# reginald-mclean/mtrl

Measured on AMD Instinct MI355X. Metric: SAC gradient-steps/sec, MT50 width-2048 batch=128/task, 1/2/4/8 MI355X, higher is better.
Workload: dtype fp32 (2xfp16 split, per-tensor power-of-two scaled, 3 fp16 MFMA products, fp32-accurate); 1 GPU; MT50 MTMHSAC-v2 width=2048 (experiments/width_scaling/mt50_mtmhsac_v2_2048.py); num_tasks=50, width=2048, batch_per_task=128, global_batch=6400, parallelism=single, precision=split2h, exec=eager

## Files before the change

### mtrl_amd/csrc/gemm_common.h

```cpp
#pragma once
#include "kernels.h"

namespace mtsac {

struct GemmSlice {
  const float* A;
  const float* B;
  float* C;
  float* db;
  int K, ldc, z;
};

template <bool TA, bool TB>
__device__ inline GemmSlice gemm_slice(const GemmParams& p) {
  GemmSlice s;
  const int S = p.splits > 1 ? p.splits : 1;
  const int zz = blockIdx.z, z = zz / S, sp = zz - z * S;
  const int k0 = sp * p.kchunk;
  s.z = z;
  s.K = S > 1 ? min(p.kchunk, p.K - k0) : p.K;
  s.A = p.A + z * p.sA + (TA ? (long long)k0 * p.lda : (long long)k0);
  s.B = p.B + z * p.sB + (TB ? (long long)k0 : (long long)k0 * p.ldb);
  if (S > 1) {
    const long long slab = (long long)p.M * p.N;
    s.C = p.ws + zz * slab;
    s.ldc = p.N;
    s.db = p.db ? p.ws + (long long)gridDim.z * slab + (long long)zz * p.N : nullptr;
  } else {
    s.C = p.C + z * p.sC;
    s.ldc = p.ldc;
    s.db = p.db ? p.db + z * p.sDb : nullptr;
  }
  return s;
}

typedef float f32x16_t __attribute__((ext_vector_type(16)));
typedef __bf16 bf16x4_t __attribute__((ext_vector_type(4)));

struct TileOut {
  float* C;
  long long ldc;
  const float* bias;
  const float* mask;
  long long ldm;
  __bf16* Cp;
  long long ldcp, pC;
  int M, N;
  bool vec;
  bool h2;
  float unscale, oscale;
};

typedef _Float16 f16x8 __attribute__((ext_vector_type(8)));

__host__ __device__ inline long long frag_off(long long n, long long k, long long ldk) {
  return (((n >> 4) * (ldk >> 5) + (k >> 5)) << 9) + (((n & 15) + 16 * ((k >> 3) & 3)) << 3) + (k & 7);
}
typedef _Float16 f16x4 __attribute__((ext_vector_type(4)));

__device__ inline void split2h_dev(float x, float s, _Float16& h, _Float16& l) {
  const float y = x * s;
  h = (_Float16)y;
  l = (_Float16)(y - (float)h);
  if (x > 0.f && h == (_Float16)0.f && l == (_Float16)0.f) l = __builtin_bit_cast(_Float16, (unsigned short)1);
}

__device__ inline int plane_exp(float bound) {
  bound *= 1.00390625f;
  if (!(bound > 0.f) || !(bound < 3.0e38f)) return 0;
  int ex;
  (void)frexpf(bound, &ex);
  return min(100, max(-100, 15 - ex));
}

__device__ inline float block_max_val(float m, float* scratch) {
#pragma unroll
  for (int o = 32; o > 0; o >>= 1) m = fmaxf(m, __shfl_xor(m, o));
  __syncthreads();
  if ((threadIdx.x & 63) == 0) scratch[threadIdx.x >> 6] = m;
  __syncthreads();
  float r = 0.f;
  for (int w = 0; w < (int)(blockDim.x + 63) / 64; ++w) r = fmaxf(r, scratch[w]);
  __syncthreads();
  return r;
}

__device__ inline float block_max_of(const float* __restrict__ v, int n, float* scratch) {
  float m = 0.f;
  for (int i = threadIdx.x; i < n; i += blockDim.x) m = fmaxf(m, v[i]);
#pragma unroll
  for (int o = 32; o > 0; o >>= 1) m = fmaxf(m, __shfl_xor(m, o));
  __syncthreads();
  if ((threadIdx.x & 63) == 0) scratch[threadIdx.x >> 6] = m;
  __syncthreads();
  float r = 0.f;
  for (int w = 0; w < (int)(blockDim.x + 63) / 64; ++w) r = fmaxf(r, scratch[w]);
  __syncthreads();
  return r;
}

__device__ inline float exp2i(int e) { return __builtin_bit_cast(float, (unsigned)(127 + e) << 23); }

__device__ inline float rec_max(const PlaneRec* r, int n, float* scratch) {
  if (r == nullptr) return 0.f;
  if (n <= 0) return exp2i(15 - r->e);
  return block_max_of(r->amax, n, scratch);
}

__device__ inline int gemm_out_exp(const SplitGemmParams& p, float* scratch) {
  const float ma = rec_max(p.ra, p.na, scratch);
  const float mb = rec_max(p.rb, p.nb, scratch);
  return plane_exp(p.kmul * ma * mb + (p.bias_in_b ? mb : 0.f));
}

__device__ inline void split3_dev(float x, __bf16& h, __bf16& m, __bf16& l) {
  h = (__bf16)x;
  const float r1 = x - (float)h;
  m = (__bf16)r1;
  l = (__bf16)(r1 - (float)m);
}

template <int EPI>
__device__ inline void store_tile32(const f32x16_t& acc, float* scr, int lane, int row0, int col0, const TileOut& o,
                                    float& omx) {
  const int lr = lane & 31, lh = lane >> 5;
#pragma unroll
  for (int r = 0; r < 16; ++r) scr[((r & 3) + 8 * (r >> 2) + 4 * lh) * 36 + lr] = acc[r];
  __builtin_amdgcn_fence(__ATOMIC_RELEASE, "wavefront");
  __builtin_amdgcn_wave_barrier();
  __builtin_amdgcn_fence(__ATOMIC_ACQUIRE, "wavefront");
  const int c4 = 4 * (lane & 7);
  const int col = col0 + c4;
#pragma unroll
  for (int q = 0; q < 4; ++q) {
    const int rr = (lane >> 3) + 8 * q;
    const int row = row0 + rr;
    if (row >= o.M) continue;
    float4 v = *reinterpret_cast<const float4*>(scr + rr * 36 + c4);
    float e[4] = {v.x, v.y, v.z, v.w};
    if (o.h2) {
#pragma unroll
      for (int j = 0; j < 4; ++j) e[j] *= o.unscale;
    }
    if (o.vec && col + 3 < o.N) {
      if (EPI == EPI_BIAS_RELU) {
        const float4 b = *reinterpret_cast<const float4*>(o.bias + col);
        e[0] = fmaxf(e[0] + b.x, 0.f); e[1] = fmaxf(e[1] + b.y, 0.f);
        e[2] = fmaxf(e[2] + b.z, 0.f); e[3] = fmaxf(e[3] + b.w, 0.f);
      }
      if (EPI == EPI_RELU_MASK) {
        const float4 mk = *reinterpret_cast<const float4*>(o.mask + (long long)row * o.ldm + col);
        e[0] = mk.x > 0.f ? e[0] : 0.f; e[1] = mk.y > 0.f ? e[1] : 0.f;
        e[2] = mk.z > 0.f ? e[2] : 0.f; e[3] = mk.w > 0.f ? e[3] : 0.f;
      }
      if (o.C) *reinterpret_cast<float4*>(o.C + (long long)row * o.ldc + col) = make_float4(e[0], e[1], e[2], e[3]);
      if (o.Cp && o.h2) {
        f16x4 h, l;
#pragma unroll
        for (int j = 0; j < 4; ++j) {
          _Float16 a, b;
          split2h_dev(e[j], o.oscale, a, b);
          h[j] = a; l[j] = b;
          omx = fmaxf(omx, fabsf(e[j]));
        }
        __bf16* cp = o.Cp + (long long)row * o.ldcp + col;
        *reinterpret_cast<f16x4*>(cp) = h;
        *reinterpret_cast<f16x4*>(cp + o.pC) = l;
      } else if (o.Cp) {
        bf16x4_t h, m, l;
#pragma unroll
        for (int j = 0; j < 4; ++j) {
          __bf16 a, b, c;
          split3_dev(e[j], a, b, c);
          h[j] = a; m[j] = b; l[j] = c;
        }
        __bf16* cp = o.Cp + (long long)row * o.ldcp + col;
        *reinterpret_cast<bf16x4_t*>(cp) = h;
        *reinterpret_cast<bf16x4_t*>(cp + o.pC) = m;
        *reinterpret_cast<bf16x4_t*>(cp + 2 * o.pC) = l;
      }
    } else {
#pragma unroll
      for (int j = 0; j < 4; ++j) {
        const int cc = col + j;
        if (cc >= o.N) continue;
        float x = e[j];
        if (EPI == EPI_BIAS_RELU) x = fmaxf(x + o.bias[cc], 0.f);
        if (EPI == EPI_RELU_MASK) x = o.mask[(long long)row * o.ldm + cc] > 0.f ? x : 0.f;
        if (o.C) o.C[(long long)row * o.ldc + cc] = x;
        if (o.Cp && o.h2) {
          _Float16 a, b;
          split2h_dev(x, o.oscale, a, b);
          omx = fmaxf(omx, fabsf(x));
          reinterpret_cast<_Float16*>(o.Cp)[(long long)row * o.ldcp + cc] = a;
          reinterpret_cast<_Float16*>(o.Cp)[(long long)row * o.ldcp + cc + o.pC] = b;
        } else if (o.Cp) {
          __bf16 a, b, c;
          split3_dev(x, a, b, c);
          __bf16* cp = o.Cp + (long long)row * o.ldcp + cc;
          cp[0] = a;
          cp[o.pC] = b;
          cp[2 * o.pC] = c;
        }
      }
    }
  }
  __builtin_amdgcn_fence(__ATOMIC_RELEASE, "wavefront");
  __builtin_amdgcn_wave_barrier();
  __builtin_amdgcn_fence(__ATOMIC_ACQUIRE, "wavefront");
}

}
```

### mtrl_amd/csrc/gemm_x3p_impl.h

```cpp
#pragma once
#include <algorithm>

#include "gemm_common.h"

namespace mtsac {

typedef f32x16_t f32x16;
typedef __bf16 bf16x8 __attribute__((ext_vector_type(8)));
typedef short i16x4 __attribute__((ext_vector_type(4)));
typedef short i16x8 __attribute__((ext_vector_type(8)));

namespace x3pk {

constexpr int BK = 32;

typedef __attribute__((address_space(3))) void lds_void;

__device__ inline void glds16(const void* src, unsigned lds_addr) {
  asm volatile("s_mov_b32 m0, %1\n\ts_nop 0\n\tglobal_load_lds_dwordx4 %0, off" ::"v"(src),
               "s"(__builtin_amdgcn_readfirstlane(lds_addr))
               : "memory");
}
template <int R, bool KM, int KS, int NP = 3>
struct Oper {
  static constexpr int PLANE = R * KS * 2;
  static constexpr int BYTES = NP * PLANE;
  static constexpr int NJ = NP * PLANE / 1024;
  static constexpr int ROWB = KM ? 2 * R : 2 * KS;
  static constexpr int RPI = 1024 / ROWB;
  static constexpr int LPR = ROWB / 16;
  static constexpr int PER_PLANE = NJ / NP;
  static_assert(!KM || LPR >= 16, "k-major swizzle needs >= 16 chunks per row");

  __device__ static inline int pchunk(int irow, int c) {
    if (KM) return c ^ (4 * (irow & 3));
    return KS == 32 ? (c ^ ((irow >> 2) & 3)) : (c ^ ((irow >> 3) & 1));
  }

  __device__ static inline void dma(const __bf16* __restrict__ base, long long ld, long long ps, int r0, int nrows,
                                    int k0, unsigned lds, int first, int stride) {
#pragma unroll
    for (int j = first; j < NJ; j += stride) dma_one(base, ld, ps, r0, nrows, k0, lds, j);
  }

  __device__ static inline void dma_one(const __bf16* __restrict__ base, long long ld, long long ps, int r0, int nrows,
                                        int k0, unsigned lds, int j) {
    const int lane = threadIdx.x & 63;
    {
      const int q = j / PER_PLANE;
      const int ib = (j % PER_PLANE) * RPI;
      const int irow = ib + lane / LPR;
      const int c = pchunk(irow, lane % LPR);
      const __bf16* src;
      if (KM) {
        int col = r0 + 8 * c;
        const int last = ((nrows + 7) & ~7) - 8;
        col = col < last ? col : last;
        src = base + q * ps + (long long)(k0 + irow) * ld + col;
      } else {
        int row = r0 + irow;
        row = row < nrows ? row : nrows - 1;
        src = base + q * ps + (long long)row * ld + k0 + 8 * c;
      }
      glds16(src, lds + q * PLANE + ib * ROWB);
    }
  }

  __device__ static inline const __bf16* dma_src(const __bf16* __restrict__ base, long long ld, long long ps, int r0,
                                                 int nrows, int k0, int j) {
    static_assert(KM, "k-major images only");
    const int lane = threadIdx.x & 63;
    const int q = j / PER_PLANE;
    const int irow = (j % PER_PLANE) * RPI + lane / LPR;
    int col = r0 + 8 * pchunk(irow, lane % LPR);
    const int last = ((nrows + 7) & ~7) - 8;
    col = col < last ? col : last;
    return base + q * ps + (long long)(k0 + irow) * ld + col;
  }
  __device__ static inline unsigned dma_dst(int j) { return (j / PER_PLANE) * PLANE + (j % PER_PLANE) * RPI * ROWB; }

  __device__ static inline bf16x8 frag(const char* lds, int q, int rb, int ks, int lane) {
    const char* pl = lds + q * PLANE;
    if (!KM) {
      const int r = rb + (lane & 31);
      const int o = r * ROWB + 16 * pchunk(r, (KS / 8 == 4 ? 2 * ks : 0) + (lane >> 5));
      return *reinterpret_cast<const bf16x8*>(pl + o);
    } else {
      const int G = lane >> 4, i = lane & 15, qq = i >> 2, p = i & 3;
      const int m = rb + 16 * (G & 1) + 4 * p;
      const int c = m >> 3, inb = 8 * (p & 1);
      const int k0 = 16 * ks + 8 * (G >> 1) + qq;
      const int o0 = k0 * ROWB + 16 * pchunk(k0, c) + inb;
      const int o1 = (k0 + 4) * ROWB + 16 * pchunk(k0 + 4, c) + inb;
      const i16x4 lo = __builtin_amdgcn_ds_read_tr16_b64_v4i16((__attribute__((address_space(3))) i16x4*)(pl + o0));
      const i16x4 hi = __builtin_amdgcn_ds_read_tr16_b64_v4i16((__attribute__((address_space(3))) i16x4*)(pl + o1));
      const i16x8 v = {lo[0], lo[1], lo[2], lo[3], hi[0], hi[1], hi[2], hi[3]};
      return __builtin_bit_cast(bf16x8, v);
    }
  }
};

template <int BM_, int BN_, int WM_, int WN_, int STAGES_, int KS_, int TAG = 0>
struct Geo {
  static constexpr int BM = BM_, BN = BN_, WM = WM_, WN = WN_, STAGES = STAGES_, KS = KS_;
  static constexpr int NW = WM * WN, NTH = 64 * NW;
  static constexpr int TI = BM / WM / 32, TJ = BN / WN / 32;
};

template <int V>
struct IntC {
  static constexpr int value = V;
};

template <class G, bool AKM, bool BKM, int EPI, bool PLANES_OUT, int NP = 3, bool FIN = false, bool PIPE = false,
          int ABL = 0>
__global__ __launch_bounds__(G::NTH, 1) void gemm_x3p_kernel(SplitGemmParams p) {
  using OA = Oper<G::BM, AKM, G::KS, NP>;
  using OB = Oper<G::BN, BKM, G::KS, NP>;
  constexpr int STAGE = OA::BYTES + OB::BYTES;
  constexpr int DMA_LO = (OA::NJ + OB::NJ) / G::NW, DMA_X = (OA::NJ + OB::NJ) % G::NW;
  constexpr int RING = PIPE ? (NP == 2 ? 6 : 4) : G::STAGES;
  static_assert(RING * STAGE + (FIN ? 16 : 0) <= 160 * 1024, "LDS");
  __shared__ __attribute__((aligned(16))) char smem[RING * STAGE + (FIN ? 16 : 0)];
  char* lds = smem;
  const unsigned lds_base = (unsigned)(unsigned long long)(lds_void*)smem;

  const int ny = (p.N + G::BN - 1) / G::BN, nx = (p.M + G::BM - 1) / G::BM;
  const int t = threadIdx.x, lane = t & 63;
  const int wave = __builtin_amdgcn_readfirstlane(t >> 6);
  const int wm = (wave % G::WM) * (G::BM / G::WM), wn = (wave / G::WM) * (G::BN / G::WN);
  const int fb = (G::NW - (OA::NJ % G::NW) + wave) % G::NW;
  constexpr int PIECES = DMA_LO + (DMA_X ? 1 : 0);
  constexpr int SLOTS = (G::KS / 16) * G::TI * G::TJ;

  f32x16 acc[G::TI][G::TJ];

  auto kloop = [&](const __bf16* __restrict__ A, const __bf16* __restrict__ B, int m0, int n0, int nk) {
    auto stage = [&](int s, int k0) {
      const unsigned st = lds_base + s * STAGE;
      OA::dma(A, p.lda, p.pA, m0, p.M, k0, st, wave, G::NW);
      OB::dma(B, p.ldb, p.pB, n0, p.N, k0, st + OA::BYTES, fb, G::NW);
    };
    auto piece = [&](int s, int k0, int q) {
      const unsigned st = lds_base + s * STAGE;
      const int jg = wave + q * G::NW;
      if (jg < OA::NJ)
        OA::dma_one(A, p.lda, p.pA, m0, p.M, k0, st, jg);
      else if (jg - OA::NJ < OB::NJ)
        OB::dma_one(B, p.ldb, p.pB, n0, p.N, k0, st + OA::BYTES, jg - OA::NJ);
    };
#pragma unroll
    for (int i = 0; i < G::TI; ++i)
#pragma unroll
      for (int j = 0; j < G::TJ; ++j) acc[i][j] = f32x16{0};

#pragma unroll
    for (int s = 0; s < G::STAGES - 1; ++s)
      if (s < nk) stage(s, s * G::KS);

    for (int kt = 0; kt < nk; ++kt) {
      const int younger = min(G::STAGES - 2, nk - 1 - kt);
      const bool more = DMA_X != 0 && wave < DMA_X;
      if (younger >= 3) {
        if (more) asm volatile("s_waitcnt vmcnt(%0)" ::"n"(3 * (DMA_LO + 1)) : "memory");
        else asm volatile("s_waitcnt vmcnt(%0)" ::"n"(3 * DMA_LO) : "memory");
      } else if (younger == 2) {
        if (more) asm volatile("s_waitcnt vmcnt(%0)" ::"n"(2 * (DMA_LO + 1)) : "memory");
        else asm volatile("s_waitcnt vmcnt(%0)" ::"n"(2 * DMA_LO) : "memory");
      } else if (younger == 1) {
        if (more) asm volatile("s_waitcnt vmcnt(%0)" ::"n"(DMA_LO + 1) : "memory");
        else asm volatile("s_waitcnt vmcnt(%0)" ::"n"(DMA_LO) : "memory");
      } else {
        asm volatile("s_waitcnt vmcnt(0)" ::: "memory");
      }
      __builtin_amdgcn_s_barrier();
      __builtin_amdgcn_sched_barrier(0);
      const bool refill = kt + G::STAGES - 1 < nk && !(p.dbg & 1);
      const int rs = (kt + G::STAGES - 1) % G::STAGES, rk = (kt + G::STAGES - 1) * G::KS;
      if (refill && (p.dbg & 8)) stage(rs, rk);
      const bool spread = refill && !(p.dbg & 8);
      const char* cur = lds + (kt % G::STAGES) * STAGE;
#pragma unroll
      for (int ks = 0; ks < G::KS / 16; ++ks) {
        bf16x8 a[G::TI][NP], b[G::TJ][NP];
#pragma unroll
        for (int i = 0; i < G::TI; ++i)
#pragma unroll
          for (int q = 0; q < NP; ++q) a[i][q] = OA::frag(cur, q, wm + 32 * i, ks, lane);
#pragma unroll
        for (int j = 0; j < G::TJ; ++j)
#pragma unroll
          for (int q = 0; q < NP; ++q) b[j][q] = OB::frag(cur + OA::BYTES, q, wn + 32 * j, ks, lane);
        if (p.dbg & 2) {
#pragma unroll
          for (int i = 0; i < G::TI; ++i)
#pragma unroll
            for (int j = 0; j < G::TJ; ++j) acc[i][j][0] += (float)a[i][0][0] + (float)b[j][2][7];
          if (spread && ks == 0)
#pragma unroll
            for (int q = 0; q < PIECES; ++q) piece(rs, rk, q);
          continue;
        }
#pragma unroll
        for (int i = 0; i < G::TI; ++i)
#pragma unroll
          for (int j = 0; j < G::TJ; ++j) {
            const int slot = (ks * G::TI + i) * G::TJ + j;
            if (spread) {
#pragma unroll
              for (int q = slot * PIECES / SLOTS; q < (slot + 1) * PIECES / SLOTS; ++q) piece(rs, rk, q);
            }
            f32x16 c = acc[i][j];
            if constexpr (NP == 2) {
              typedef _Float16 h8 __attribute__((ext_vector_type(8)));
              c = __builtin_amdgcn_mfma_f32_32x32x16_f16(__builtin_bit_cast(h8, a[i][0]), __builtin_bit_cast(h8, b[j][1]), c, 0, 0, 0);
              c = __builtin_amdgcn_mfma_f32_32x32x16_f16(__builtin_bit_cast(h8, a[i][1]), __builtin_bit_cast(h8, b[j][0]), c, 0, 0, 0);
              c = __builtin_amdgcn_mfma_f32_32x32x16_f16(__builtin_bit_cast(h8, a[i][0]), __builtin_bit_cast(h8, b[j][0]), c, 0, 0, 0);
              acc[i][j] = c;
              continue;
            }
            if constexpr (NP == 3) {
              c = __builtin_amdgcn_mfma_f32_32x32x16_bf16(a[i][1], b[j][1], c, 0, 0, 0);
              c = __builtin_amdgcn_mfma_f32_32x32x16_bf16(a[i][0], b[j][2], c, 0, 0, 0);
              c = __builtin_amdgcn_mfma_f32_32x32x16_bf16(a[i][2], b[j][0], c, 0, 0, 0);
              c = __builtin_amdgcn_mfma_f32_32x32x16_bf16(a[i][0], b[j][1], c, 0, 0, 0);
              c = __builtin_amdgcn_mfma_f32_32x32x16_bf16(a[i][1], b[j][0], c, 0, 0, 0);
            }
            c = __builtin_amdgcn_mfma_f32_32x32x16_bf16(a[i][0], b[j][0], c, 0, 0, 0);
            acc[i][j] = c;
          }
      }
    }
  };

  auto epilogue = [&](int z, int zz, bool raw, int m0, int n0) {
    TileOut o{};
    if (raw) {
      o.C = p.ws + (long long)zz * p.M * p.N;
      o.ldc = p.N;
    } else {
      o.C = p.C ? p.C + z * p.sC : nullptr;
      o.ldc = p.ldc;
    }
    o.bias = (EPI == EPI_BIAS_RELU) ? p.bias + z * p.sBias : nullptr;
    o.mask = (EPI == EPI_RELU_MASK) ? p.mask + z * p.sMask : nullptr;
    o.ldm = p.ldm;
    o.Cp = (PLANES_OUT && !raw) ? p.Cp + z * p.sCp : nullptr;
    o.ldcp = p.ldcp;
    o.pC = p.pC;
    o.M = p.M;
    o.N = p.N;
    o.vec = (p.N % 4 == 0) && (o.ldc % 4 == 0) && (EPI != EPI_RELU_MASK || p.ldm % 4 == 0) &&
            (!PLANES_OUT || p.ldcp % 4 == 0);
    o.h2 = NP == 2;
    o.unscale = o.oscale = 1.f;
    __builtin_amdgcn_s_barrier();
    float* mscr = reinterpret_cast<float*>(smem) + G::NW * (32 * 36);
    if constexpr (NP == 2) {
      o.unscale = exp2i(-p.ra->e) * exp2i(-p.rb->e);
      if (o.Cp) {
        const int ec = gemm_out_exp(p, mscr);
        o.oscale = exp2i(ec);
        if (blockIdx.x == 0 && t == 0) p.rc->e = ec;
      }
    }
    float omx = 0.f;
    float* scr = reinterpret_cast<float*>(smem) + wave * (32 * 36);
#pragma unroll
    for (int i = 0; i < G::TI; ++i)
#pragma unroll
      for (int j = 0; j < G::TJ; ++j) store_tile32<EPI>(acc[i][j], scr, lane, m0 + wm + 32 * i, n0 + wn + 32 * j, o, omx);
    if constexpr (NP == 2) {
      if (o.Cp) {
        const float m = block_max_val(omx, mscr);
        if (t == 0 && blockIdx.x < PLANE_REC_PARTS) p.rc->amax[blockIdx.x] = m;
      }
    }
  };

  int lin = blockIdx.x;
  if (!(p.dbg & 4)) {
    const int n = gridDim.x, q8 = n / 8, r8 = n % 8, x = lin % 8;
    lin = (x < r8 ? x * (q8 + 1) : r8 * (q8 + 1) + (x - r8) * q8) + lin / 8;
  }
  const int S = p.splits > 1 ? p.splits : 1;
  const int sp0 = FIN ? lin % S : 0;
  if (FIN) lin /= S;
  const int by = lin % ny, bx = (lin / ny) % nx;
  const int z = FIN ? lin / (ny * nx) : lin / (ny * nx) / S;
  const int sp = FIN ? sp0 : lin / (ny * nx) - z * S;
  const int zz = z * S + sp;
  const long long k0 = (long long)sp * p.kchunk;
  const int nks = (S > 1 ? min(p.kchunk, p.K - (int)k0) : p.K) / G::KS;
  const int m0 = bx * G::BM, n0 = by * G::BN;
  if constexpr (PIPE) {
    static_assert(AKM && BKM && G::KS == 16 && (NP == 2 || NP == 3), "the k-major weight-grad form");
    static_assert(OA::NJ % G::NW == 0, "every wave's first pieces are A's, the rest B's");
    static_assert(RING >= 3, "ring depth");
    constexpr int D = RING;
    constexpr int QA = OA::NJ / G::NW;
    struct Frag {
      bf16x8 a[G::TI][NP], b[G::TJ][NP];
    };
    const __bf16* __restrict__ A = p.A + z * p.sA + k0 * p.lda;
    const __bf16* __restrict__ B = p.B + z * p.sB + k0 * p.ldb;
    const int nk = nks;
    const bool extra = DMA_X != 0 && wave < DMA_X;
    const __bf16* src[PIECES];
    unsigned dst[PIECES];
#pragma unroll
    for (int q = 0; q < PIECES; ++q) {
      const int jg = wave + q * G::NW;
      if (q < QA) {
        src[q] = OA::dma_src(A, p.lda, p.pA, m0, p.M, D * G::KS, jg);
        dst[q] = OA::dma_dst(jg);
      } else {
        const int jb = jg - OA::NJ < OB::NJ ? jg - OA::NJ : 0;
        src[q] = OB::dma_src(B, p.ldb, p.pB, n0, p.N, D * G::KS, jb);
        dst[q] = OA::BYTES + OB::dma_dst(jb);
      }
    }
    const long long inc_a = (long long)G::KS * p.lda, inc_b = (long long)G::KS * p.ldb;
    auto piece = [&](unsigned st, int q) __attribute__((always_inline)) {
      if (q < DMA_LO || extra) glds16(src[q], st + dst[q]);
      src[q] += q < QA ? inc_a : inc_b;
    };
    auto wait_c = [&](auto Y) __attribute__((always_inline)) {
      constexpr int y = decltype(Y)::value;
      if (DMA_X != 0 && extra) asm volatile("s_waitcnt vmcnt(%0)" ::"n"(y * (DMA_LO + 1)) : "memory");
      else asm volatile("s_waitcnt vmcnt(%0)" ::"n"(y * DMA_LO) : "memory");
    };
    auto wait_rt = [&](int y) __attribute__((always_inline)) {
      if constexpr (D - 1 >= 5) if (y >= 5) return wait_c(IntC<5>{});
      if constexpr (D - 1 >= 4) if (y == 4) return wait_c(IntC<4>{});
      if constexpr (D - 1 >= 3) if (y == 3) return wait_c(IntC<3>{});
      if (y == 2) return wait_c(IntC<2>{});
      if (y == 1) return wait_c(IntC<1>{});
      return wait_c(IntC<0>{});
    };
    static_assert(D - 1 <= 5 && (D - 1) * (DMA_LO + 1) < 64, "vmcnt range");
    auto load = [&](Frag& f, const char* st) __attribute__((always_inline)) {
#pragma unroll
      for (int i = 0; i < G::TI; ++i)
#pragma unroll
        for (int q = 0; q < NP; ++q) f.a[i][q] = OA::frag(st, q, wm + 32 * i, 0, lane);
#pragma unroll
      for (int j = 0; j < G::TJ; ++j)
#pragma unroll
        for (int q = 0; q < NP; ++q) f.b[j][q] = OB::frag(st + OA::BYTES, q, wn + 32 * j, 0, lane);
    };

#pragma unroll
    for (int i = 0; i < G::TI; ++i)
#pragma unroll
      for (int j = 0; j < G::TJ; ++j) acc[i][j] = f32x16{0};

#pragma unroll
    for (int s = 0; s < D; ++s)
      if (s < nk) {
        const unsigned st = lds_base + s * STAGE;
        OA::dma(A, p.lda, p.pA, m0, p.M, s * G::KS, st, wave, G::NW);
        OB::dma(B, p.ldb, p.pB, n0, p.N, s * G::KS, st + OA::BYTES, fb, G::NW);
      }
    wait_rt(min(D, nk) - 1);
    __builtin_amdgcn_s_barrier();
    __builtin_amdgcn_sched_barrier(0);
    Frag f0, f1;
    load(f0, lds);

    int slot = 0, nslot = 1 % D;
    auto step = [&](int kt, Frag& cur, Frag& nxt, auto MAINC) __attribute__((always_inline)) {
      constexpr bool MAIN = decltype(MAINC)::value != 0;
      if constexpr (MAIN) wait_c(IntC<D - 2>{});
      else wait_rt(min(D - 2, max(0, nk - 2 - kt)));
      asm volatile("s_waitcnt lgkmcnt(0)" ::: "memory");
      __builtin_amdgcn_s_barrier();
      __builtin_amdgcn_sched_barrier(0);
      const bool refill = !(ABL & 1) && (MAIN || kt + D < nk);
      const bool pre = MAIN || kt + 1 < nk;
      const unsigned rst = lds_base + slot * STAGE;
      const char* nst = lds + nslot * STAGE;
      if ((ABL & 8) && refill) {
#pragma unroll
        for (int q = 0; q < PIECES; ++q) piece(rst, q);
      }
#pragma unroll
      for (int i = 0; i < G::TI; ++i)
#pragma unroll
        for (int j = 0; j < G::TJ; ++j) {
          const int g = i * G::TJ + j;
          if (!(ABL & 8) && refill) {
#pragma unroll
            for (int q = g * PIECES / SLOTS; q < (g + 1) * PIECES / SLOTS; ++q) piece(rst, q);
          }
          if constexpr ((ABL & 2) != 0) {
            acc[i][j][0] += (float)cur.a[i][0][0] + (float)cur.b[j][NP - 1][7];
          } else {
            f32x16 c = acc[i][j];
            if constexpr (NP == 2) {
              typedef _Float16 h8 __attribute__((ext_vector_type(8)));
              c = __builtin_amdgcn_mfma_f32_32x32x16_f16(__builtin_bit_cast(h8, cur.a[i][0]), __builtin_bit_cast(h8, cur.b[j][1]), c, 0, 0, 0);
              c = __builtin_amdgcn_mfma_f32_32x32x16_f16(__builtin_bit_cast(h8, cur.a[i][1]), __builtin_bit_cast(h8, cur.b[j][0]), c, 0, 0, 0);
              c = __builtin_amdgcn_mfma_f32_32x32x16_f16(__builtin_bit_cast(h8, cur.a[i][0]), __builtin_bit_cast(h8, cur.b[j][0]), c, 0, 0, 0);
            } else {
              c = __builtin_amdgcn_mfma_f32_32x32x16_bf16(cur.a[i][1], cur.b[j][1], c, 0, 0, 0);
              c = __builtin_amdgcn_mfma_f32_32x32x16_bf16(cur.a[i][0], cur.b[j][2], c, 0, 0, 0);
              c = __builtin_amdgcn_mfma_f32_32x32x16_bf16(cur.a[i][2], cur.b[j][0], c, 0, 0, 0);
              c = __builtin_amdgcn_mfma_f32_32x32x16_bf16(cur.a[i][0], cur.b[j][1], c, 0, 0, 0);
              c = __builtin_amdgcn_mfma_f32_32x32x16_bf16(cur.a[i][1], cur.b[j][0], c, 0, 0, 0);
              c = __builtin_amdgcn_mfma_f32_32x32x16_bf16(cur.a[i][0], cur.b[j][0], c, 0, 0, 0);
            }
            acc[i][j] = c;
          }
          if (g == 0 && pre) load(nxt, nst);
          __builtin_amdgcn_sched_barrier(0);
        }
      slot = nslot;
      nslot = nslot + 1 == D ? 0 : nslot + 1;
    };
    int kt = 0;
    for (; kt + D + 1 < nk; kt += 2) {
      step(kt, f0, f1, IntC<1>{});
      step(kt + 1, f1, f0, IntC<1>{});
    }
    for (; kt < nk; kt += 2) {
      step(kt, f0, f1, IntC<0>{});
      if (kt + 1 < nk) step(kt + 1, f1, f0, IntC<0>{});
    }
  } else {
    kloop(p.A + z * p.sA + (AKM ? k0 * p.lda : k0), p.B + z * p.sB + (BKM ? k0 * p.ldb : k0), m0, n0, nks);
  }
  epilogue(z, zz, S > 1, m0, n0);
  if constexpr (FIN) {
    asm volatile("s_waitcnt vmcnt(0)" ::: "memory");
    __syncthreads();
    int* last = reinterpret_cast<int*>(smem + RING * STAGE);
    const int tile = lin;
    if (t == 0) {
      __builtin_amdgcn_fence(__ATOMIC_RELEASE, "agent");
      asm volatile("s_waitcnt vmcnt(0)" ::: "memory");
      const int tk = __hip_atomic_fetch_add(p.cnt + tile, 1, __ATOMIC_RELAXED, __HIP_MEMORY_SCOPE_AGENT);
      const int me = tk == S - 1;
      if (me) __hip_atomic_store(p.cnt + tile, 0, __ATOMIC_RELAXED, __HIP_MEMORY_SCOPE_AGENT);
      *last = me;
    }
    __syncthreads();
    if (*last == 0) return;
    if (t == 0) {
      __builtin_amdgcn_fence(__ATOMIC_ACQUIRE, "agent");
      asm volatile("s_waitcnt vmcnt(0)" ::: "memory");
    }
    __syncthreads();
    const long long slab = (long long)p.M * p.N;
    const float* w = p.ws + (long long)z * S * slab;
    float* c = p.C + z * p.sC;
    constexpr int Q = G::BN / 4;
    constexpr int U = 8;
    static_assert(G::BM * Q % (G::NTH * U) == 0, "reduce tiling");
    for (int e0 = t; e0 < G::BM * Q; e0 += G::NTH * U) {
      float4 a[U];
      long long off[U];
      bool ok[U];
#pragma unroll
      for (int u = 0; u < U; ++u) {
        const int e = e0 + u * G::NTH, r = m0 + e / Q, cc = n0 + 4 * (e % Q);
        ok[u] = r < p.M && cc < p.N;
        off[u] = (long long)r * p.N + cc;
        if (ok[u]) a[u] = *reinterpret_cast<const float4*>(w + off[u]);
      }
      for (int s = 1; s < S; ++s) {
#pragma unroll
        for (int u = 0; u < U; ++u)
          if (ok[u]) {
            const float4 v = *reinterpret_cast<const float4*>(w + s * slab + off[u]);
            a[u].x += v.x; a[u].y += v.y; a[u].z += v.z; a[u].w += v.w;
          }
      }
#pragma unroll
      for (int u = 0; u < U; ++u)
        if (ok[u]) {
          const int e = e0 + u * G::NTH, r = m0 + e / Q, cc = n0 + 4 * (e % Q);
          *reinterpret_cast<float4*>(c + (long long)r * p.ldc + cc) = a[u];
        }
    }
  }
}

using GeoSmall = Geo<128, 128, 2, 2, 3, 32>;
using GeoWide = Geo<256, 128, 4, 2, 2, 32>;
using GeoWide16 = Geo<256, 128, 4, 2, 4, 16>;
using GeoBig16 = Geo<256, 256, 2, 4, 3, 16>;
using GeoSmall16 = Geo<128, 128, 2, 2, 3, 16>;
using GeoBig16In = Geo<256, 256, 2, 4, 3, 16, 1>;
using GeoTall224 = Geo<224, 256, 1, 8, 3, 16>;
using GeoTall224In = Geo<224, 256, 1, 8, 3, 16, 1>;

template <class G, bool AKM, bool BKM, int NP>
void launch_x3p_np(const SplitGemmParams& p, int epi, dim3 grid, hipStream_t st) {
  const bool planes = p.Cp != nullptr;
  const dim3 block(G::NTH);
  if constexpr (AKM && BKM && NP == 3 && G::STAGES * (G::BM + G::BN) * G::KS * 2 * 3 + 16 <= 160 * 1024) {
    if (epi == EPI_STORE && !planes && p.cnt != nullptr && p.splits > 1) {
      hipLaunchKernelGGL((gemm_x3p_kernel<G, true, true, EPI_STORE, false, 3, true>), grid, block, 0, st, p);
      return;
    }
  }
  if constexpr (AKM && BKM && (NP == 2 || NP == 3) && G::BM == 256 && G::BN == 128 && G::WM == 4 && G::WN == 2 &&
                G::KS == 16) {
    if (epi == EPI_STORE && !planes && !(p.dbg & 16)) {
      const int abl = NP != 2 ? 0 : (p.dbg & 1) ? 1 : (p.dbg & 2) ? 2 : (p.dbg & 8);
      if (abl == 1) hipLaunchKernelGGL((gemm_x3p_kernel<G, true, true, EPI_STORE, false, NP, false, true, NP == 2 ? 1 : 0>), grid, block, 0, st, p);
      else if (abl == 2) hipLaunchKernelGGL((gemm_x3p_kernel<G, true, true, EPI_STORE, false, NP, false, true, NP == 2 ? 2 : 0>), grid, block, 0, st, p);
      else if (abl == 8) hipLaunchKernelGGL((gemm_x3p_kernel<G, true, true, EPI_STORE, false, NP, false, true, NP == 2 ? 8 : 0>), grid, block, 0, st, p);
      else hipLaunchKernelGGL((gemm_x3p_kernel<G, true, true, EPI_STORE, false, NP, false, true, 0>), grid, block, 0, st, p);
      return;
    }
  }
  if (epi == EPI_BIAS_RELU) {
    if (planes) hipLaunchKernelGGL((gemm_x3p_kernel<G, AKM, BKM, EPI_BIAS_RELU, true, NP>), grid, block, 0, st, p);
    else hipLaunchKernelGGL((gemm_x3p_kernel<G, AKM, BKM, EPI_BIAS_RELU, false, NP>), grid, block, 0, st, p);
  } else if (epi == EPI_RELU_MASK) {
    if (planes) hipLaunchKernelGGL((gemm_x3p_kernel<G, AKM, BKM, EPI_RELU_MASK, true, NP>), grid, block, 0, st, p);
    else hipLaunchKernelGGL((gemm_x3p_kernel<G, AKM, BKM, EPI_RELU_MASK, false, NP>), grid, block, 0, st, p);
  } else {
    if (planes) hipLaunchKernelGGL((gemm_x3p_kernel<G, AKM, BKM, EPI_STORE, true, NP>), grid, block, 0, st, p);
    else hipLaunchKernelGGL((gemm_x3p_kernel<G, AKM, BKM, EPI_STORE, false, NP>), grid, block, 0, st, p);
  }
}

template <class G, bool AKM, bool BKM>
void launch_x3p_v(const SplitGemmParams& p, int epi, dim3 grid, hipStream_t st) {
  if (p.np == 1) launch_x3p_np<G, AKM, BKM, 1>(p, epi, grid, st);
  else if (p.np == 2) launch_x3p_np<G, AKM, BKM, 2>(p, epi, grid, st);
  else launch_x3p_np<G, AKM, BKM, 3>(p, epi, grid, st);
}

template <class G, int MASK>
void launch_forms(const SplitGemmParams& p, int epi, dim3 grid, hipStream_t st) {
  const int form = (p.a_kmajor ? 1 : 0) | (p.b_kmajor ? 2 : 0);
#define X3P_FORM(F, AK, BK)                      \
  if constexpr (((MASK >> F) & 1) != 0)          \
    if (form == F) {                             \
      launch_x3p_v<G, AK, BK>(p, epi, grid, st); \
      return;                                    \
    }
  X3P_FORM(0, false, false)
  X3P_FORM(1, true, false)
  X3P_FORM(2, false, true)
  X3P_FORM(3, true, true)
#undef X3P_FORM
}

}

#define X3P_UNIT(NAME, GEO, MASK)                                           \
  void NAME(const SplitGemmParams& p, int epi, dim3 grid, hipStream_t st) { \
    x3pk::launch_forms<x3pk::GEO, MASK>(p, epi, grid, st);                  \
  }
void x3p_unit_g0(const SplitGemmParams&, int, dim3, hipStream_t);
void x3p_unit_g1(const SplitGemmParams&, int, dim3, hipStream_t);
void x3p_unit_g2(const SplitGemmParams&, int, dim3, hipStream_t);
void x3p_unit_g3f0(const SplitGemmParams&, int, dim3, hipStream_t);
void x3p_unit_g3f1(const SplitGemmParams&, int, dim3, hipStream_t);
void x3p_unit_g3f2(const SplitGemmParams&, int, dim3, hipStream_t);
void x3p_unit_g3f3(const SplitGemmParams&, int, dim3, hipStream_t);
void x3p_unit_g4(const SplitGemmParams&, int, dim3, hipStream_t);
void x3p_unit_g3in(const SplitGemmParams&, int, dim3, hipStream_t);
void x3p_unit_g5(const SplitGemmParams&, int, dim3, hipStream_t);
void x3p_unit_g5in(const SplitGemmParams&, int, dim3, hipStream_t);

}
```

Baseline: 226.0 SAC gradient-steps/sec.

## Use 16x16x32 f16 MFMA for split2h k-major weight-gradient GEMM

Adds a 16x16x32 f16 MFMA path for the two-plane split2h k-major weight-gradient GEMM, and makes it the default. The path uses transposed LDS reads (ds_read_tr16) over a new paired-stage swizzle and consumes two K stages per pipeline step. The epilogue reassembles the 16x16 accumulators into 32x32 tiles through scratch before storing. The goal is higher MFMA throughput and fewer fragment loads than the 32x32x16 instruction gives, at the cost of more accumulator registers, a different swizzle and a more complex pipeline.

```diff
diff --git a/mtrl_amd/csrc/gemm_common.h b/mtrl_amd/csrc/gemm_common.h
--- a/mtrl_amd/csrc/gemm_common.h
+++ b/mtrl_amd/csrc/gemm_common.h
@@ -121,11 +121,7 @@
 }
 
 template <int EPI>
-__device__ inline void store_tile32(const f32x16_t& acc, float* scr, int lane, int row0, int col0, const TileOut& o,
-                                    float& omx) {
-  const int lr = lane & 31, lh = lane >> 5;
-#pragma unroll
-  for (int r = 0; r < 16; ++r) scr[((r & 3) + 8 * (r >> 2) + 4 * lh) * 36 + lr] = acc[r];
+__device__ inline void store_tile32_rows(float* scr, int lane, int row0, int col0, const TileOut& o, float& omx) {
   __builtin_amdgcn_fence(__ATOMIC_RELEASE, "wavefront");
   __builtin_amdgcn_wave_barrier();
   __builtin_amdgcn_fence(__ATOMIC_ACQUIRE, "wavefront");
@@ -210,4 +206,13 @@
   __builtin_amdgcn_fence(__ATOMIC_ACQUIRE, "wavefront");
 }
 
-}
+template <int EPI>
+__device__ inline void store_tile32(const f32x16_t& acc, float* scr, int lane, int row0, int col0, const TileOut& o,
+                                    float& omx) {
+  const int lr = lane & 31, lh = lane >> 5;
+#pragma unroll
+  for (int r = 0; r < 16; ++r) scr[((r & 3) + 8 * (r >> 2) + 4 * lh) * 36 + lr] = acc[r];
+  store_tile32_rows<EPI>(scr, lane, row0, col0, o, omx);
+}
+
+}
diff --git a/mtrl_amd/csrc/gemm_x3p_impl.h b/mtrl_amd/csrc/gemm_x3p_impl.h
--- a/mtrl_amd/csrc/gemm_x3p_impl.h
+++ b/mtrl_amd/csrc/gemm_x3p_impl.h
@@ -6,6 +6,7 @@
 namespace mtsac {
 
 typedef f32x16_t f32x16;
+typedef float f32x4 __attribute__((ext_vector_type(4)));
 typedef __bf16 bf16x8 __attribute__((ext_vector_type(8)));
 typedef short i16x4 __attribute__((ext_vector_type(4)));
 typedef short i16x8 __attribute__((ext_vector_type(8)));
@@ -21,7 +22,7 @@
                "s"(__builtin_amdgcn_readfirstlane(lds_addr))
                : "memory");
 }
-template <int R, bool KM, int KS, int NP = 3>
+template <int R, bool KM, int KS, int NP = 3, bool SW8 = false>
 struct Oper {
   static constexpr int PLANE = R * KS * 2;
   static constexpr int BYTES = NP * PLANE;
@@ -33,6 +34,7 @@
   static_assert(!KM || LPR >= 16, "k-major swizzle needs >= 16 chunks per row");
 
   __device__ static inline int pchunk(int irow, int c) {
+    if (KM && SW8) return c ^ (4 * (irow & 3)) ^ (2 * ((irow >> 3) & 1));
     if (KM) return c ^ (4 * (irow & 3));
     return KS == 32 ? (c ^ ((irow >> 2) & 3)) : (c ^ ((irow >> 3) & 1));
   }
@@ -98,6 +100,21 @@
       return __builtin_bit_cast(bf16x8, v);
     }
   }
+
+  __device__ static inline bf16x8 frag16(const char* lds, int pair, int q, int rb, int lane) {
+    static_assert(KM && KS == 16 && SW8, "the paired k-major image");
+    const int G = lane >> 4, i = lane & 15, qq = i >> 2, p = i & 3;
+    const int m = rb + 4 * p;
+    const int c = m >> 3, inb = 8 * (p & 1);
+    const int k0 = 8 * (G & 1) + qq;
+    const char* pl = lds + (G >> 1) * pair + q * PLANE;
+    const int o0 = k0 * ROWB + 16 * pchunk(k0, c) + inb;
+    const int o1 = (k0 + 4) * ROWB + 16 * pchunk(k0 + 4, c) + inb;
+    const i16x4 lo = __builtin_amdgcn_ds_read_tr16_b64_v4i16((__attribute__((address_space(3))) i16x4*)(pl + o0));
+    const i16x4 hi = __builtin_amdgcn_ds_read_tr16_b64_v4i16((__attribute__((address_space(3))) i16x4*)(pl + o1));
+    const i16x8 v = {lo[0], lo[1], lo[2], lo[3], hi[0], hi[1], hi[2], hi[3]};
+    return __builtin_bit_cast(bf16x8, v);
+  }
 };
 
 template <int BM_, int BN_, int WM_, int WN_, int STAGES_, int KS_, int TAG = 0>
@@ -113,10 +130,13 @@
 };
 
 template <class G, bool AKM, bool BKM, int EPI, bool PLANES_OUT, int NP = 3, bool FIN = false, bool PIPE = false,
-          int ABL = 0>
+          int ABL = 0, int MS = 32>
 __global__ __launch_bounds__(G::NTH, 1) void gemm_x3p_kernel(SplitGemmParams p) {
-  using OA = Oper<G::BM, AKM, G::KS, NP>;
-  using OB = Oper<G::BN, BKM, G::KS, NP>;
+  static_assert(MS == 32 || (MS == 16 && AKM && BKM && G::KS == 16 && NP == 2 && EPI == EPI_STORE && !PLANES_OUT &&
+                             !FIN && G::BM / G::WM == 64 && G::BN / G::WN == 64 && G::STAGES % 2 == 0),
+                "16x16x32: the split2h k-major weight-grad form only");
+  using OA = Oper<G::BM, AKM, G::KS, NP, MS == 16>;
+  using OB = Oper<G::BN, BKM, G::KS, NP, MS == 16>;
   constexpr int STAGE = OA::BYTES + OB::BYTES;
   constexpr int DMA_LO = (OA::NJ + OB::NJ) / G::NW, DMA_X = (OA::NJ + OB::NJ) % G::NW;
   constexpr int RING = PIPE ? (NP == 2 ? 6 : 4) : G::STAGES;
@@ -134,6 +154,71 @@
   constexpr int SLOTS = (G::KS / 16) * G::TI * G::TJ;
 
   f32x16 acc[G::TI][G::TJ];
+  constexpr int T16 = 4, GROUPS16 = T16 * T16 / 2;
+  constexpr int STAGE2 = 2 * STAGE;
+  f32x4 acc16[T16][T16];
+  struct Frag16 {
+    bf16x8 a[T16][2], b[T16][2];
+  };
+  auto load16 = [&](Frag16& f, const char* st) __attribute__((always_inline)) {
+    if constexpr (MS == 16) {
+#pragma unroll
+      for (int i = 0; i < T16; ++i)
+#pragma unroll
+        for (int q = 0; q < 2; ++q) f.a[i][q] = OA::frag16(st, STAGE, q, wm + 16 * i, lane);
+#pragma unroll
+      for (int j = 0; j < T16; ++j)
+#pragma unroll
+        for (int q = 0; q < 2; ++q) f.b[j][q] = OB::frag16(st + OA::BYTES, STAGE, q, wn + 16 * j, lane);
+    }
+  };
+  auto group16 = [&](const Frag16& f, int g) __attribute__((always_inline)) {
+    typedef _Float16 h8 __attribute__((ext_vector_type(8)));
+    const int i = g / 2, j = 2 * (g % 2);
+    if constexpr ((ABL & 2) != 0) {
+      acc16[i][j][0] += (float)f.a[i][0][0] + (float)f.b[j][1][7];
+      acc16[i][j + 1][0] += (float)f.a[i][1][0] + (float)f.b[j + 1][1][7];
+    } else {
+      const h8 ah = __builtin_bit_cast(h8, f.a[i][0]), al = __builtin_bit_cast(h8, f.a[i][1]);
+      const h8 bh0 = __builtin_bit_cast(h8, f.b[j][0]), bl0 = __builtin_bit_cast(h8, f.b[j][1]);
+      const h8 bh1 = __builtin_bit_cast(h8, f.b[j + 1][0]), bl1 = __builtin_bit_cast(h8, f.b[j + 1][1]);
+      f32x4 c0 = acc16[i][j], c1 = acc16[i][j + 1];
+      c0 = __builtin_amdgcn_mfma_f32_16x16x32_f16(ah, bl0, c0, 0, 0, 0);
+      c1 = __builtin_amdgcn_mfma_f32_16x16x32_f16(ah, bl1, c1, 0, 0, 0);
+      c0 = __builtin_amdgcn_mfma_f32_16x16x32_f16(al, bh0, c0, 0, 0, 0);
+      c1 = __builtin_amdgcn_mfma_f32_16x16x32_f16(al, bh1, c1, 0, 0, 0);
+      c0 = __builtin_amdgcn_mfma_f32_16x16x32_f16(ah, bh0, c0, 0, 0, 0);
+      c1 = __builtin_amdgcn_mfma_f32_16x16x32_f16(ah, bh1, c1, 0, 0, 0);
+      acc16[i][j] = c0;
+      acc16[i][j + 1] = c1;
+    }
+  };
+  auto kloop16 = [&](const __bf16* __restrict__ A, const __bf16* __restrict__ B, int m0, int n0, int nk) {
+    auto stage2 = [&](int s2, int k0) {
+#pragma unroll
+      for (int h = 0; h < 2; ++h) {
+        const unsigned st = lds_base + s2 * STAGE2 + h * STAGE;
+        OA::dma(A, p.lda, p.pA, m0, p.M, k0 + h * G::KS, st, wave, G::NW);
+        OB::dma(B, p.ldb, p.pB, n0, p.N, k0 + h * G::KS, st + OA::BYTES, fb, G::NW);
+      }
+    };
+#pragma unroll
+    for (int i = 0; i < T16; ++i)
+#pragma unroll
+      for (int j = 0; j < T16; ++j) acc16[i][j] = f32x4{0};
+    stage2(0, 0);
+    for (int kt = 0; kt < nk; kt += 2) {
+      asm volatile("s_waitcnt vmcnt(0)" ::: "memory");
+      __builtin_amdgcn_s_barrier();
+      __builtin_amdgcn_sched_barrier(0);
+      const int s2 = (kt >> 1) & 1;
+      if (kt + 2 < nk) stage2(s2 ^ 1, (kt + 2) * G::KS);
+      Frag16 f;
+      load16(f, lds + s2 * STAGE2);
+#pragma unroll
+      for (int g = 0; g < GROUPS16; ++g) group16(f, g);
+    }
+  };
 
   auto kloop = [&](const __bf16* __restrict__ A, const __bf16* __restrict__ B, int m0, int n0, int nk) {
     auto stage = [&](int s, int k0) {
@@ -266,10 +351,27 @@
     }
     float omx = 0.f;
     float* scr = reinterpret_cast<float*>(smem) + wave * (32 * 36);
-#pragma unroll
-    for (int i = 0; i < G::TI; ++i)
-#pragma unroll
-      for (int j = 0; j < G::TJ; ++j) store_tile32<EPI>(acc[i][j], scr, lane, m0 + wm + 32 * i, n0 + wn + 32 * j, o, omx);
+    if constexpr (MS == 16) {
+#pragma unroll
+      for (int i = 0; i < T16 / 2; ++i)
+#pragma unroll
+        for (int j = 0; j < T16 / 2; ++j) {
+#pragma unroll
+          for (int bi = 0; bi < 2; ++bi)
+#pragma unroll
+            for (int bj = 0; bj < 2; ++bj)
+#pragma unroll
+              for (int r = 0; r < 4; ++r)
+                scr[(16 * bi + 4 * (lane >> 4) + r) * 36 + 16 * bj + (lane & 15)] = acc16[2 * i + bi][2 * j + bj][r];
+          store_tile32_rows<EPI>(scr, lane, m0 + wm + 32 * i, n0 + wn + 32 * j, o, omx);
+        }
+    } else {
+#pragma unroll
+      for (int i = 0; i < G::TI; ++i)
+#pragma unroll
+        for (int j = 0; j < G::TJ; ++j)
+          store_tile32<EPI>(acc[i][j], scr, lane, m0 + wm + 32 * i, n0 + wn + 32 * j, o, omx);
+    }
     if constexpr (NP == 2) {
       if (o.Cp) {
         const float m = block_max_val(omx, mscr);
@@ -339,94 +441,156 @@
       return wait_c(IntC<0>{});
     };
     static_assert(D - 1 <= 5 && (D - 1) * (DMA_LO + 1) < 64, "vmcnt range");
-    auto load = [&](Frag& f, const char* st) __attribute__((always_inline)) {
-#pragma unroll
-      for (int i = 0; i < G::TI; ++i)
-#pragma unroll
-        for (int q = 0; q < NP; ++q) f.a[i][q] = OA::frag(st, q, wm + 32 * i, 0, lane);
-#pragma unroll
-      for (int j = 0; j < G::TJ; ++j)
-#pragma unroll
-        for (int q = 0; q < NP; ++q) f.b[j][q] = OB::frag(st + OA::BYTES, q, wn + 32 * j, 0, lane);
-    };
-
-#pragma unroll
-    for (int i = 0; i < G::TI; ++i)
-#pragma unroll
-      for (int j = 0; j < G::TJ; ++j) acc[i][j] = f32x16{0};
-
-#pragma unroll
-    for (int s = 0; s < D; ++s)
-      if (s < nk) {
-        const unsigned st = lds_base + s * STAGE;
-        OA::dma(A, p.lda, p.pA, m0, p.M, s * G::KS, st, wave, G::NW);
-        OB::dma(B, p.ldb, p.pB, n0, p.N, s * G::KS, st + OA::BYTES, fb, G::NW);
-      }
-    wait_rt(min(D, nk) - 1);
-    __builtin_amdgcn_s_barrier();
-    __builtin_amdgcn_sched_barrier(0);
-    Frag f0, f1;
-    load(f0, lds);
-
-    int slot = 0, nslot = 1 % D;
-    auto step = [&](int kt, Frag& cur, Frag& nxt, auto MAINC) __attribute__((always_inline)) {
-      constexpr bool MAIN = decltype(MAINC)::value != 0;
-      if constexpr (MAIN) wait_c(IntC<D - 2>{});
-      else wait_rt(min(D - 2, max(0, nk - 2 - kt)));
-      asm volatile("s_waitcnt lgkmcnt(0)" ::: "memory");
+    if constexpr (MS == 16) {
+      static_assert(D % 2 == 0 && D >= 6, "pairs of ring stages, one pair in flight");
+#pragma unroll
+      for (int i = 0; i < T16; ++i)
+#pragma unroll
+        for (int j = 0; j < T16; ++j) acc16[i][j] = f32x4{0};
+#pragma unroll
+      for (int s = 0; s < D; ++s)
+        if (s < nk) {
+          const unsigned st = lds_base + s * STAGE;
+          OA::dma(A, p.lda, p.pA, m0, p.M, s * G::KS, st, wave, G::NW);
+          OB::dma(B, p.ldb, p.pB, n0, p.N, s * G::KS, st + OA::BYTES, fb, G::NW);
+        }
+      wait_rt(min(D, nk) - 2);
       __builtin_amdgcn_s_barrier();
       __builtin_amdgcn_sched_barrier(0);
-      const bool refill = !(ABL & 1) && (MAIN || kt + D < nk);
-      const bool pre = MAIN || kt + 1 < nk;
-      const unsigned rst = lds_base + slot * STAGE;
-      const char* nst = lds + nslot * STAGE;
-      if ((ABL & 8) && refill) {
-#pragma unroll
-        for (int q = 0; q < PIECES; ++q) piece(rst, q);
-      }
-#pragma unroll
-      for (int i = 0; i < G::TI; ++i)
-#pragma unroll
-        for (int j = 0; j < G::TJ; ++j) {
-          const int g = i * G::TJ + j;
+      Frag16 f0, f1;
+      load16(f0, lds);
+
+      int slot = 0, nslot = 1;
+      auto step = [&](int kt, Frag16& cur, Frag16& nxt, auto MAINC) __attribute__((always_inline)) {
+        constexpr bool MAIN = decltype(MAINC)::value != 0;
+        if constexpr (MAIN) wait_c(IntC<D - 4>{});
+        else wait_rt(min(D - 4, max(0, nk - 4 - kt)));
+        asm volatile("s_waitcnt lgkmcnt(0)" ::: "memory");
+        __builtin_amdgcn_s_barrier();
+        __builtin_amdgcn_sched_barrier(0);
+        const bool refill = !(ABL & 1) && (MAIN || kt + D < nk);
+        const bool pre = MAIN || kt + 2 < nk;
+        const unsigned rst = lds_base + slot * STAGE2;
+        const char* nst = lds + nslot * STAGE2;
+        if ((ABL & 8) && refill) {
+#pragma unroll
+          for (int q = 0; q < 2 * PIECES; ++q) piece(rst + (q / PIECES) * STAGE, q % PIECES);
+        }
+#pragma unroll
+        for (int g = 0; g < GROUPS16; ++g) {
           if (!(ABL & 8) && refill) {
 #pragma unroll
-            for (int q = g * PIECES / SLOTS; q < (g + 1) * PIECES / SLOTS; ++q) piece(rst, q);
+            for (int q = g * 2 * PIECES / GROUPS16; q < (g + 1) * 2 * PIECES / GROUPS16; ++q)
+              piece(rst + (q / PIECES) * STAGE, q % PIECES);
           }
-          if constexpr ((ABL & 2) != 0) {
-            acc[i][j][0] += (float)cur.a[i][0][0] + (float)cur.b[j][NP - 1][7];
-          } else {
-            f32x16 c = acc[i][j];
-            if constexpr (NP == 2) {
-              typedef _Float16 h8 __attribute__((ext_vector_type(8)));
-              c = __builtin_amdgcn_mfma_f32_32x32x16_f16(__builtin_bit_cast(h8, cur.a[i][0]), __builtin_bit_cast(h8, cur.b[j][1]), c, 0, 0, 0);
-              c = __builtin_amdgcn_mfma_f32_32x32x16_f16(__builtin_bit_cast(h8, cur.a[i][1]), __builtin_bit_cast(h8, cur.b[j][0]), c, 0, 0, 0);
-              c = __builtin_amdgcn_mfma_f32_32x32x16_f16(__builtin_bit_cast(h8, cur.a[i][0]), __builtin_bit_cast(h8, cur.b[j][0]), c, 0, 0, 0);
-            } else {
-              c = __builtin_amdgcn_mfma_f32_32x32x16_bf16(cur.a[i][1], cur.b[j][1], c, 0, 0, 0);
-              c = __builtin_amdgcn_mfma_f32_32x32x16_bf16(cur.a[i][0], cur.b[j][2], c, 0, 0, 0);
-              c = __builtin_amdgcn_mfma_f32_32x32x16_bf16(cur.a[i][2], cur.b[j][0], c, 0, 0, 0);
-              c = __builtin_amdgcn_mfma_f32_32x32x16_bf16(cur.a[i][0], cur.b[j][1], c, 0, 0, 0);
-              c = __builtin_amdgcn_mfma_f32_32x32x16_bf16(cur.a[i][1], cur.b[j][0], c, 0, 0, 0);
-              c = __builtin_amdgcn_mfma_f32_32x32x16_bf16(cur.a[i][0], cur.b[j][0], c, 0, 0, 0);
-            }
-            acc[i][j] = c;
-          }
-          if (g == 0 && pre) load(nxt, nst);
+          group16(cur, g);
+          if (g == 0 && pre) load16(nxt, nst);
           __builtin_amdgcn_sched_barrier(0);
         }
-      slot = nslot;
-      nslot = nslot + 1 == D ? 0 : nslot + 1;
-    };
-    int kt = 0;
-    for (; kt + D + 1 < nk; kt += 2) {
-      step(kt, f0, f1, IntC<1>{});
-      step(kt + 1, f1, f0, IntC<1>{});
-    }
-    for (; kt < nk; kt += 2) {
-      step(kt, f0, f1, IntC<0>{});
-      if (kt + 1 < nk) step(kt + 1, f1, f0, IntC<0>{});
-    }
+        slot = nslot;
+        nslot = nslot + 1 == D / 2 ? 0 : nslot + 1;
+      };
+      int kt = 0;
+      for (; kt + D + 3 < nk; kt += 4) {
+        step(kt, f0, f1, IntC<1>{});
+        step(kt + 2, f1, f0, IntC<1>{});
+      }
+      for (; kt < nk; kt += 4) {
+        step(kt, f0, f1, IntC<0>{});
+        if (kt + 2 < nk) step(kt + 2, f1, f0, IntC<0>{});
+      }
+    } else {
+      auto load = [&](Frag& f, const char* st) __attribute__((always_inline)) {
+#pragma unroll
+        for (int i = 0; i < G::TI; ++i)
+#pragma unroll
+          for (int q = 0; q < NP; ++q) f.a[i][q] = OA::frag(st, q, wm + 32 * i, 0, lane);
+#pragma unroll
+        for (int j = 0; j < G::TJ; ++j)
+#pragma unroll
+          for (int q = 0; q < NP; ++q) f.b[j][q] = OB::frag(st + OA::BYTES, q, wn + 32 * j, 0, lane);
+      };
+
+#pragma unroll
+      for (int i = 0; i < G::TI; ++i)
+#pragma unroll
+        for (int j = 0; j < G::TJ; ++j) acc[i][j] = f32x16{0};
+
+#pragma unroll
+      for (int s = 0; s < D; ++s)
+        if (s < nk) {
+          const unsigned st = lds_base + s * STAGE;
+          OA::dma(A, p.lda, p.pA, m0, p.M, s * G::KS, st, wave, G::NW);
+          OB::dma(B, p.ldb, p.pB, n0, p.N, s * G::KS, st + OA::BYTES, fb, G::NW);
+        }
+      wait_rt(min(D, nk) - 1);
+      __builtin_amdgcn_s_barrier();
+      __builtin_amdgcn_sched_barrier(0);
+      Frag f0, f1;
+      load(f0, lds);
+
+      int slot = 0, nslot = 1 % D;
+      auto step = [&](int kt, Frag& cur, Frag& nxt, auto MAINC) __attribute__((always_inline)) {
+        constexpr bool MAIN = decltype(MAINC)::value != 0;
+        if constexpr (MAIN) wait_c(IntC<D - 2>{});
+        else wait_rt(min(D - 2, max(0, nk - 2 - kt)));
+        asm volatile("s_waitcnt lgkmcnt(0)" ::: "memory");
+        __builtin_amdgcn_s_barrier();
+        __builtin_amdgcn_sched_barrier(0);
+        const bool refill = !(ABL & 1) && (MAIN || kt + D < nk);
+        const bool pre = MAIN || kt + 1 < nk;
+        const unsigned rst = lds_base + slot * STAGE;
+        const char* nst = lds + nslot * STAGE;
+        if ((ABL & 8) && refill) {
+#pragma unroll
+          for (int q = 0; q < PIECES; ++q) piece(rst, q);
+        }
+#pragma unroll
+        for (int i = 0; i < G::TI; ++i)
+#pragma unroll
+          for (int j = 0; j < G::TJ; ++j) {
+            const int g = i * G::TJ + j;
+            if (!(ABL & 8) && refill) {
+#pragma unroll
+              for (int q = g * PIECES / SLOTS; q < (g + 1) * PIECES / SLOTS; ++q) piece(rst, q);
+            }
+            if constexpr ((ABL & 2) != 0) {
+              acc[i][j][0] += (float)cur.a[i][0][0] + (float)cur.b[j][NP - 1][7];
+            } else {
+              f32x16 c = acc[i][j];
+              if constexpr (NP == 2) {
+                typedef _Float16 h8 __attribute__((ext_vector_type(8)));
+                c = __builtin_amdgcn_mfma_f32_32x32x16_f16(__builtin_bit_cast(h8, cur.a[i][0]), __builtin_bit_cast(h8, cur.b[j][1]), c, 0, 0, 0);
+                c = __builtin_amdgcn_mfma_f32_32x32x16_f16(__builtin_bit_cast(h8, cur.a[i][1]), __builtin_bit_cast(h8, cur.b[j][0]), c, 0, 0, 0);
+                c = __builtin_amdgcn_mfma_f32_32x32x16_f16(__builtin_bit_cast(h8, cur.a[i][0]), __builtin_bit_cast(h8, cur.b[j][0]), c, 0, 0, 0);
+              } else {
+                c = __builtin_amdgcn_mfma_f32_32x32x16_bf16(cur.a[i][1], cur.b[j][1], c, 0, 0, 0);
+                c = __builtin_amdgcn_mfma_f32_32x32x16_bf16(cur.a[i][0], cur.b[j][2], c, 0, 0, 0);
+                c = __builtin_amdgcn_mfma_f32_32x32x16_bf16(cur.a[i][2], cur.b[j][0], c, 0, 0, 0);
+                c = __builtin_amdgcn_mfma_f32_32x32x16_bf16(cur.a[i][0], cur.b[j][1], c, 0, 0, 0);
+                c = __builtin_amdgcn_mfma_f32_32x32x16_bf16(cur.a[i][1], cur.b[j][0], c, 0, 0, 0);
+                c = __builtin_amdgcn_mfma_f32_32x32x16_bf16(cur.a[i][0], cur.b[j][0], c, 0, 0, 0);
+              }
+              acc[i][j] = c;
+            }
+            if (g == 0 && pre) load(nxt, nst);
+            __builtin_amdgcn_sched_barrier(0);
+          }
+        slot = nslot;
+        nslot = nslot + 1 == D ? 0 : nslot + 1;
+      };
+      int kt = 0;
+      for (; kt + D + 1 < nk; kt += 2) {
+        step(kt, f0, f1, IntC<1>{});
+        step(kt + 1, f1, f0, IntC<1>{});
+      }
+      for (; kt < nk; kt += 2) {
+        step(kt, f0, f1, IntC<0>{});
+        if (kt + 1 < nk) step(kt + 1, f1, f0, IntC<0>{});
+      }
+    }
+  } else if constexpr (MS == 16) {
+    kloop16(p.A + z * p.sA + k0 * p.lda, p.B + z * p.sB + k0 * p.ldb, m0, n0, nks);
   } else {
     kloop(p.A + z * p.sA + (AKM ? k0 * p.lda : k0), p.B + z * p.sB + (BKM ? k0 * p.ldb : k0), m0, n0, nks);
   }
@@ -495,6 +659,8 @@
 using GeoTall224 = Geo<224, 256, 1, 8, 3, 16>;
 using GeoTall224In = Geo<224, 256, 1, 8, 3, 16, 1>;
 
+constexpr bool X3P_MFMA16_DEFAULT = true;
+
 template <class G, bool AKM, bool BKM, int NP>
 void launch_x3p_np(const SplitGemmParams& p, int epi, dim3 grid, hipStream_t st) {
   const bool planes = p.Cp != nullptr;
@@ -507,6 +673,17 @@
   }
   if constexpr (AKM && BKM && (NP == 2 || NP == 3) && G::BM == 256 && G::BN == 128 && G::WM == 4 && G::WN == 2 &&
                 G::KS == 16) {
+    if constexpr (NP == 2) {
+      if (epi == EPI_STORE && !planes && X3P_MFMA16_DEFAULT != ((p.dbg & 32) != 0)) {
+        const int abl = (p.dbg & 16) ? 16 : (p.dbg & 1) ? 1 : (p.dbg & 2) ? 2 : (p.dbg & 8);
+        if (abl == 16) hipLaunchKernelGGL((gemm_x3p_kernel<G, true, true, EPI_STORE, false, 2, false, false, 0, 16>), grid, block, 0, st, p);
+        else if (abl == 1) hipLaunchKernelGGL((gemm_x3p_kernel<G, true, true, EPI_STORE, false, 2, false, true, 1, 16>), grid, block, 0, st, p);
+        else if (abl == 2) hipLaunchKernelGGL((gemm_x3p_kernel<G, true, true, EPI_STORE, false, 2, false, true, 2, 16>), grid, block, 0, st, p);
+        else if (abl == 8) hipLaunchKernelGGL((gemm_x3p_kernel<G, true, true, EPI_STORE, false, 2, false, true, 8, 16>), grid, block, 0, st, p);
+        else hipLaunchKernelGGL((gemm_x3p_kernel<G, true, true, EPI_STORE, false, 2, false, true, 0, 16>), grid, block, 0, st, p);
+        return;
+      }
+    }
     if (epi == EPI_STORE && !planes && !(p.dbg & 16)) {
       const int abl = NP != 2 ? 0 : (p.dbg & 1) ? 1 : (p.dbg & 2) ? 2 : (p.dbg & 8);
       if (abl == 1) hipLaunchKernelGGL((gemm_x3p_kernel<G, true, true, EPI_STORE, false, NP, false, true, NP == 2 ? 1 : 0>), grid, block, 0, st, p);
```

Result: no change. 228.1 SAC gradient-steps/sec (median of 6 runs) (+0.9%).
